# imjaegyun/Traffic-Context-Augmented-Vehicle-Trajectory-Prediction-Framework-Using-Multimodal-LLM

Hardware: AMD Instinct MI355X
Metric: trajectories/sec (higher is better)
Workload: dtype f16

## Files before the change

### traffic-context-augmented-vehicle-trajectory-prediction-framework-using-multimodal-llm_amd/csrc/attention.hip

```cpp
#include "common.hpp"
#include "philox.hpp"

namespace tcavt {

__device__ __forceinline__ f16x8 cvt8_f16(const float* v) {
  f16x8 o;
#pragma unroll
  for (int i = 0; i < 8; ++i) o[i] = static_cast<_Float16>(v[i]);
  return o;
}

__device__ __forceinline__ void halves(float x, float& lo, float& hi) {
  const auto r = __builtin_amdgcn_permlane32_swap(__float_as_uint(x), __float_as_uint(x), false, false);
  lo = __uint_as_float(r[0]);
  hi = __uint_as_float(r[1]);
}

__device__ __forceinline__ unsigned int bf16pair_to_f16pair(unsigned int k0_bits, unsigned int k1_bits) {
  const float a = fminf(fmaxf(__uint_as_float(k0_bits << 16), -65504.f), 65504.f);
  const float b = fminf(fmaxf(__uint_as_float(k1_bits << 16), -65504.f), 65504.f);
  const unsigned short ha = __builtin_bit_cast(unsigned short, static_cast<_Float16>(a));
  const unsigned short hb = __builtin_bit_cast(unsigned short, static_cast<_Float16>(b));
  return static_cast<unsigned int>(ha) | (static_cast<unsigned int>(hb) << 16);
}

template <int MAXT, bool F16>
__global__ __launch_bounds__(MAXT) void attn_causal_gqa_kernel(const bf16_t* __restrict__ qkv,
                                                              bf16_t* __restrict__ out,
                                                              const int* __restrict__ kv_len_p,
                                                              int L, int Lp, int nq, int nkv,
                                                              float scale_log2e, int ot_bytes,
                                                              float* __restrict__ lse = nullptr) {
  extern __shared__ __attribute__((aligned(16))) char smem[];
  const int group = nq / nkv;
  const int b = blockIdx.x / nkv, kvh = blockIdx.x % nkv;
  const int lane = threadIdx.x & 63;
  const int wave = __builtin_amdgcn_readfirstlane(threadIdx.x >> 6);
  const int ld = (nq + 2 * nkv) * 64;
  const int koff = nq * 64 + kvh * 64, voff = (nq + nkv) * 64 + kvh * 64;
  const int vstride = Lp + 4;
  char* Ks = smem;
  bf16_t* Vt = reinterpret_cast<bf16_t*>(smem + Lp * 128);
  const int ot_off = (Lp * 128 + 64 * (Lp + 4) * 2 + 15) & ~15;
  const bf16_t* base = qkv + (long)b * L * ld;

  const int head = kvh * group + (wave % group);
  const int qb0 = wave / group;
  const int r = lane & 31, hh = lane >> 5;
  const int nqb = (L + 31) >> 5;
  const int npair = (nqb + 1) >> 1;
  auto block_of = [&](int bi) {
    const int pr = qb0 + 2 * (bi >> 1);
    if (pr >= npair) return -1;
    const int qb = (bi & 1) ? nqb - 1 - pr : pr;
    return ((bi & 1) && qb == pr) ? -1 : qb;
  };
  auto load_q = [&](int qb, bf16x8 (&qf)[4]) {
    const int qrow = min(qb * 32 + r, L - 1);
#pragma unroll
    for (int s = 0; s < 4; ++s)
      qf[s] = *reinterpret_cast<const bf16x8*>(base + (long)qrow * ld + head * 64 + s * 16 + hh * 8);
  };
  constexpr int NPRE = 4;
  bf16x8 qpre[NPRE][4];
#pragma unroll
  for (int bi = 0; bi < NPRE; ++bi) {
    const int qb = block_of(bi);
    load_q(qb < 0 ? 0 : qb, qpre[bi]);
  }

  const int nthreads = blockDim.x;
  constexpr int KIT = 4, VIT = 2;
  auto stage_k = [&](int idx, const u32x4& v) {
    const int row = idx >> 3, c = idx & 7;
    *reinterpret_cast<u32x4*>(Ks + row * 128 + ((c ^ ((row >> 1) & 7)) << 4)) = v;
  };
  auto stage_v = [&](int idx, const u32x4& a, const u32x4& bb) {
    const int kp = idx >> 3, c = idx & 7;
    const int r0 = 2 * kp;
#pragma unroll
    for (int e = 0; e < 4; ++e) {
      unsigned int lo, hi;
      if constexpr (F16) {
        lo = (a[e] & 0xffffu) | (bb[e] << 16);
        hi = (a[e] >> 16) | (bb[e] & 0xffff0000u);
      } else {
        lo = bf16pair_to_f16pair(a[e] & 0xffffu, bb[e] & 0xffffu);
        hi = bf16pair_to_f16pair(a[e] >> 16, bb[e] >> 16);
      }
      *reinterpret_cast<unsigned int*>(Vt + (c * 8 + 2 * e) * vstride + r0) = lo;
      *reinterpret_cast<unsigned int*>(Vt + (c * 8 + 2 * e + 1) * vstride + r0) = hi;
    }
  };
  const u32x4 zero4 = {0u, 0u, 0u, 0u};
  auto load_k = [&](int idx) {
    const int row = min(idx >> 3, L - 1), c = idx & 7;
    return *reinterpret_cast<const u32x4*>(base + (long)row * ld + koff + c * 8);
  };
  auto load_v = [&](int idx, int which) {
    const int rr = min(2 * (idx >> 3) + which, L - 1), c = idx & 7;
    return *reinterpret_cast<const u32x4*>(base + (long)rr * ld + voff + c * 8);
  };
  auto krow_ok = [&](int idx) { return (idx >> 3) < L; };
  auto vrow_ok = [&](int idx, int which) { return 2 * (idx >> 3) + which < L; };
  {
    u32x4 kreg[KIT], va[VIT], vb[VIT];
#pragma unroll
    for (int it = 0; it < KIT; ++it) kreg[it] = load_k(threadIdx.x + it * nthreads);
#pragma unroll
    for (int it = 0; it < VIT; ++it) {
      va[it] = load_v(threadIdx.x + it * nthreads, 0);
      vb[it] = load_v(threadIdx.x + it * nthreads, 1);
    }
#pragma unroll
    for (int it = 0; it < KIT; ++it) {
      const int idx = threadIdx.x + it * nthreads;
      if (idx < Lp * 8) stage_k(idx, krow_ok(idx) ? kreg[it] : zero4);
    }
#pragma unroll
    for (int it = 0; it < VIT; ++it) {
      const int idx = threadIdx.x + it * nthreads;
      if (idx < (Lp >> 1) * 8) stage_v(idx, vrow_ok(idx, 0) ? va[it] : zero4, vrow_ok(idx, 1) ? vb[it] : zero4);
    }
  }
  for (int idx = threadIdx.x + KIT * nthreads; idx < Lp * 8; idx += nthreads)
    stage_k(idx, krow_ok(idx) ? load_k(idx) : zero4);
  for (int idx = threadIdx.x + VIT * nthreads; idx < (Lp >> 1) * 8; idx += nthreads)
    stage_v(idx, vrow_ok(idx, 0) ? load_v(idx, 0) : zero4, vrow_ok(idx, 1) ? load_v(idx, 1) : zero4);
  __syncthreads();

  const int kv_len = min(kv_len_p[b], L);
  const int kv_tiles = (kv_len + 31) >> 5;
  const int kswz = (r >> 1) & 7;

  auto do_block = [&](int qb, const bf16x8 (&qf)[4]) {
    const int qi = qb * 32 + r;
    f32x16 o0, o1;
#pragma unroll
    for (int i = 0; i < 16; ++i) { o0[i] = 0.f; o1[i] = 0.f; }
    float mrun = -1e30f, lrun = 0.f;

    const int ntile = min(qb + 1, kv_tiles);
    for (int kt = 0; kt < ntile; ++kt) {
      f32x16 sacc;
#pragma unroll
      for (int i = 0; i < 16; ++i) sacc[i] = 0.f;
      const char* krow = Ks + (kt * 32 + r) * 128;
#pragma unroll
      for (int s = 0; s < 4; ++s) {
        const bf16x8 kf = *reinterpret_cast<const bf16x8*>(krow + (((2 * s + hh) ^ kswz) << 4));
        if constexpr (F16)
          sacc = __builtin_amdgcn_mfma_f32_32x32x16_f16(__builtin_bit_cast(f16x8, kf), __builtin_bit_cast(f16x8, qf[s]), sacc, 0, 0, 0);
        else
          sacc = __builtin_amdgcn_mfma_f32_32x32x16_bf16(kf, qf[s], sacc, 0, 0, 0);
      }
      float p[16];
      float tmax = -1e30f;
      const bool full = (kt < qb) && (kt * 32 + 32 <= kv_len);
      if (full) {
        float rmax = fmaxf(fmaxf(sacc[0], sacc[1]), sacc[2]);
#pragma unroll
        for (int i = 3; i + 1 < 16; i += 2) rmax = fmaxf(fmaxf(rmax, sacc[i]), sacc[i + 1]);
        rmax = fmaxf(rmax, sacc[15]);
        { float a, b; halves(rmax, a, b); rmax = fmaxf(a, b); }
        const float mnew = fmaxf(mrun, rmax * scale_log2e);
        const float alpha = __builtin_amdgcn_exp2f(mrun - mnew);
        float psum = 0.f;
#pragma unroll
        for (int i = 0; i < 16; ++i) {
          p[i] = __builtin_amdgcn_exp2f(fmaf(sacc[i], scale_log2e, -mnew));
          psum += p[i];
        }
        { float a, b; halves(psum, a, b); psum = a + b; }
        lrun = lrun * alpha + psum;
        mrun = mnew;
#pragma unroll
        for (int i = 0; i < 16; ++i) { o0[i] *= alpha; o1[i] *= alpha; }
      } else {
#pragma unroll
        for (int i = 0; i < 16; ++i) {
          const int kk = kt * 32 + (i & 3) + 8 * (i >> 2) + 4 * hh;
          const bool ok = (kk <= qi) && (kk < kv_len);
          p[i] = ok ? sacc[i] * scale_log2e : -1e30f;
          tmax = fmaxf(tmax, p[i]);
        }
        { float a, b; halves(tmax, a, b); tmax = fmaxf(a, b); }
        const float mnew = fmaxf(mrun, tmax);
        const float alpha = __builtin_amdgcn_exp2f(mrun - mnew);
        float psum = 0.f;
#pragma unroll
        for (int i = 0; i < 16; ++i) {
          p[i] = (p[i] > -1e29f) ? __builtin_amdgcn_exp2f(p[i] - mnew) : 0.f;
          psum += p[i];
        }
        { float a, b; halves(psum, a, b); psum = a + b; }
        lrun = lrun * alpha + psum;
        mrun = mnew;
#pragma unroll
        for (int i = 0; i < 16; ++i) { o0[i] *= alpha; o1[i] *= alpha; }
      }
#pragma unroll
      for (int s2 = 0; s2 < 2; ++s2) {
        const f16x8 pf = cvt8_f16(&p[8 * s2]);
        const int kbase = kt * 32 + 16 * s2 + 4 * hh;
#pragma unroll
        for (int dt = 0; dt < 2; ++dt) {
          const bf16_t* vrow = Vt + (dt * 32 + r) * vstride + kbase;
          const u32x2 lo = *reinterpret_cast<const u32x2*>(vrow);
          const u32x2 hi = *reinterpret_cast<const u32x2*>(vrow + 8);
          const u32x4 vv = {lo[0], lo[1], hi[0], hi[1]};
          const f16x8 vf = __builtin_bit_cast(f16x8, vv);
          if (dt == 0) o0 = __builtin_amdgcn_mfma_f32_32x32x16_f16(vf, pf, o0, 0, 0, 0);
          else o1 = __builtin_amdgcn_mfma_f32_32x32x16_f16(vf, pf, o1, 0, 0, 0);
        }
      }
    }
    const float inv = lrun > 0.f ? 1.f / lrun : 0.f;
    if (lse && hh == 0 && qi < L) lse[((long)b * nq + head) * L + qi] = lrun > 0.f ? (mrun + __log2f(lrun)) * 0.6931471805599453f : 0.f;
    if (ot_bytes) {
      char* ot = smem + ot_off + wave * (32 * 144);
#pragma unroll
      for (int half = 0; half < 2; ++half) {
        const f32x16& o = half ? o1 : o0;
#pragma unroll
        for (int g = 0; g < 4; ++g)
          *reinterpret_cast<u32x2*>(ot + r * 144 + (half * 32 + 8 * g + 4 * hh) * 2) =
              u32x2{pack16x2<F16>(o[4 * g] * inv, o[4 * g + 1] * inv), pack16x2<F16>(o[4 * g + 2] * inv, o[4 * g + 3] * inv)};
      }
#pragma unroll
      for (int k = 0; k < 4; ++k) {
        const int row = (lane >> 3) + 8 * k, q = qb * 32 + row;
        const u32x4 v = *reinterpret_cast<const u32x4*>(ot + row * 144 + (lane & 7) * 16);
        if (q < L) *reinterpret_cast<u32x4*>(out + ((long)b * L + q) * (nq * 64) + head * 64 + (lane & 7) * 8) = v;
      }
      return;
    }
    bf16_t* orow = out + ((long)b * L + min(qi, L - 1)) * (nq * 64) + head * 64;
#pragma unroll
    for (int half = 0; half < 2; ++half) {
      const f32x16& o = half ? o1 : o0;
#pragma unroll
      for (int g = 0; g < 4; g += 2) {
        unsigned int a0 = pack16x2<F16>(o[4 * g] * inv, o[4 * g + 1] * inv), a1 = pack16x2<F16>(o[4 * g + 2] * inv, o[4 * g + 3] * inv);
        unsigned int b0 = pack16x2<F16>(o[4 * g + 4] * inv, o[4 * g + 5] * inv), b1 = pack16x2<F16>(o[4 * g + 6] * inv, o[4 * g + 7] * inv);
        auto s0 = __builtin_amdgcn_permlane32_swap(a0, b0, false, false);
        auto s1 = __builtin_amdgcn_permlane32_swap(a1, b1, false, false);
        if (qi < L) *reinterpret_cast<u32x4*>(orow + half * 32 + 8 * g + 8 * hh) = u32x4{s0[0], s1[0], s0[1], s1[1]};
      }
    }
  };

#pragma unroll
  for (int bi = 0; bi < NPRE; ++bi) {
    const int qb = block_of(bi);
    if (qb >= 0) do_block(qb, qpre[bi]);
  }
  for (int bi = NPRE;; ++bi) {
    if (qb0 + 2 * (bi >> 1) >= npair) break;
    const int qb = block_of(bi);
    if (qb < 0) continue;
    bf16x8 qf[4];
    load_q(qb, qf);
    do_block(qb, qf);
  }
}

struct b16 { bf16_t v; };
struct h16 { bf16_t v; };
template <typename T>
__device__ __forceinline__ float ldf(const T* p);
template <>
__device__ __forceinline__ float ldf<float>(const float* p) { return *p; }
template <>
__device__ __forceinline__ float ldf<b16>(const b16* p) { return bf16_to_f32(p->v); }
template <>
__device__ __forceinline__ float ldf<h16>(const h16* p) { return f16_to_f32(p->v); }
template <typename T>
__device__ __forceinline__ void stf(T* p, float x);
template <>
__device__ __forceinline__ void stf<float>(float* p, float x) { *p = x; }
template <>
__device__ __forceinline__ void stf<b16>(b16* p, float x) { p->v = f32_to_bf16(x); }
template <>
__device__ __forceinline__ void stf<h16>(h16* p, float x) { p->v = f32_to_f16(x); }

template <typename TI, typename TO>
__global__ __launch_bounds__(256) void mha_small_kernel(const TI* __restrict__ q, long ldq,
                                                        const TI* __restrict__ k, long ldk,
                                                        const TI* __restrict__ v, long ldv,
                                                        TO* __restrict__ out, long ldo,
                                                        const int* __restrict__ key_len, int Lq,
                                                        int Lk, int nh, int dh, float scale, DropoutP drop) {
  extern __shared__ __attribute__((aligned(16))) char smem[];
  float* sc = reinterpret_cast<float*>(smem);
  const int b = blockIdx.x / nh, h = blockIdx.x % nh;
  const int klen = key_len ? min(key_len[b], Lk) : Lk;
  const TI* qb = q + (long)b * Lq * ldq + h * dh;
  const TI* kb = k + (long)b * Lk * ldk + h * dh;
  const TI* vb = v + (long)b * Lk * ldv + h * dh;
  const int tid = threadIdx.x;

  const int lane = tid & 63, wave = tid >> 6;
  for (int ij = wave; ij < Lq * Lk; ij += 4) {
    const int i = ij / Lk, j = ij - i * Lk;
    float acc = 0.f;
    if (j < klen) {
      const TI* qr = qb + (long)i * ldq;
      const TI* kr = kb + (long)j * ldk;
      for (int d = lane; d < dh; d += 64) acc += ldf<TI>(qr + d) * ldf<TI>(kr + d);
      acc = wave_sum(acc);
    }
    if (lane == 0) sc[ij] = (j < klen) ? acc * scale : -1e30f;
  }
  __syncthreads();
  for (int i = wave; i < Lq; i += 4) {
    float* row = sc + i * Lk;
    float m = -1e30f;
    for (int j = lane; j < Lk; j += 64) m = fmaxf(m, row[j]);
    m = wave_max(m);
    float s = 0.f;
    for (int j = lane; j < Lk; j += 64) {
      const float e = (row[j] > -1e29f) ? __expf(row[j] - m) : 0.f;
      row[j] = e;
      s += e;
    }
    s = wave_sum(s);
    const float inv = s > 0.f ? 1.f / s : 0.f;
    for (int j = lane; j < Lk; j += 64) {
      float pj = row[j] * inv;
      if (drop.p > 0.f)
        pj *= dropout_one(drop, ((unsigned long long)blockIdx.x * Lq + i) * (unsigned long long)Lk + j);
      row[j] = pj;
    }
  }
  __syncthreads();
  for (int id = tid; id < Lq * dh; id += 256) {
    const int i = id / dh, d = id - i * dh;
    const float* row = sc + i * Lk;
    float acc = 0.f;
    for (int j = 0; j < klen; ++j) acc += row[j] * ldf<TI>(vb + (long)j * ldv + d);
    TO* o = out + ((long)b * Lq + i) * ldo + h * dh + d;
    stf<TO>(o, acc);
  }
}

template <typename TI, typename TO>
__global__ __launch_bounds__(256) void mha_lds_kernel(const TI* __restrict__ q, long ldq,
                                                      const TI* __restrict__ k, long ldk,
                                                      const TI* __restrict__ v, long ldv,
                                                      TO* __restrict__ out, long ldo,
                                                      const int* __restrict__ key_len, int Lq, int Lk,
                                                      int nh, int dh, float scale, DropoutP drop) {
  extern __shared__ __attribute__((aligned(16))) char smem[];
  const int ds = dh + 1;
  float* Qs = reinterpret_cast<float*>(smem);
  float* Ks = Qs + Lq * ds;
  float* Vs = Ks + Lk * ds;
  float* sc = Vs + Lk * ds;
  const int b = blockIdx.x / nh, h = blockIdx.x % nh;
  const int klen = key_len ? min(key_len[b], Lk) : Lk;
  const TI* qb = q + (long)b * Lq * ldq + h * dh;
  const TI* kb = k + (long)b * Lk * ldk + h * dh;
  const TI* vb = v + (long)b * Lk * ldv + h * dh;
  const int tid = threadIdx.x, lane = tid & 63, wave = tid >> 6;
  for (int id = tid; id < Lq * dh; id += 256) {
    const int i = id / dh, d = id - i * dh;
    Qs[i * ds + d] = ldf<TI>(qb + (long)i * ldq + d);
  }
  for (int id = tid; id < Lk * dh; id += 256) {
    const int j = id / dh, d = id - j * dh;
    Ks[j * ds + d] = ldf<TI>(kb + (long)j * ldk + d);
    Vs[j * ds + d] = ldf<TI>(vb + (long)j * ldv + d);
  }
  __syncthreads();
  for (int ij = tid; ij < Lq * Lk; ij += 256) {
    const int i = ij / Lk, j = ij - i * Lk;
    float acc = 0.f;
    if (j < klen) {
      const float* qr = Qs + i * ds;
      const float* kr = Ks + j * ds;
      for (int d = 0; d < dh; ++d) acc = fmaf(qr[d], kr[d], acc);
    }
    sc[ij] = (j < klen) ? acc * scale : -1e30f;
  }
  __syncthreads();
  for (int i = wave; i < Lq; i += 4) {
    float* row = sc + i * Lk;
    float m = -1e30f;
    for (int j = lane; j < Lk; j += 64) m = fmaxf(m, row[j]);
    m = wave_max(m);
    float s = 0.f;
    for (int j = lane; j < Lk; j += 64) {
      const float e = (row[j] > -1e29f) ? __expf(row[j] - m) : 0.f;
      row[j] = e;
      s += e;
    }
    s = wave_sum(s);
    const float inv = s > 0.f ? 1.f / s : 0.f;
    for (int j = lane; j < Lk; j += 64) {
      float pj = row[j] * inv;
      if (drop.p > 0.f)
        pj *= dropout_one(drop, ((unsigned long long)blockIdx.x * Lq + i) * (unsigned long long)Lk + j);
      row[j] = pj;
    }
  }
  __syncthreads();
  for (int id = tid; id < Lq * dh; id += 256) {
    const int i = id / dh, d = id - i * dh;
    const float* row = sc + i * Lk;
    float acc = 0.f;
    for (int j = 0; j < klen; ++j) acc = fmaf(row[j], Vs[j * ds + d], acc);
    TO* o = out + ((long)b * Lq + i) * ldo + h * dh + d;
    stf<TO>(o, acc);
  }
}

}

using namespace tcavt;

extern "C" int tcavt_attn_causal_gqa(const void* qkv, void* out, const int32_t* kv_len, int B, int L,
                                     int nq, int nkv, float scale, int dtype16, tcavt_stream_t stream) {
  return tcavt_attn_causal_gqa_lse(qkv, out, nullptr, kv_len, B, L, nq, nkv, scale, dtype16, stream);
}

extern "C" int tcavt_attn_causal_gqa_lse(const void* qkv, void* out, float* lse, const int32_t* kv_len, int B, int L,
                                         int nq, int nkv, float scale, int dtype16, tcavt_stream_t stream) {
  TCAVT_CHECK_ARG(qkv && out && kv_len, "attn_causal_gqa: null pointer");
  TCAVT_CHECK_ARG(is16(dtype16), "attn_causal_gqa: dtype16 must be TCAVT_BF16 or TCAVT_F16");
  TCAVT_CHECK_ARG(B > 0 && L > 0 && L <= 544, "attn_causal_gqa: L=%d must be in [1, 544]", L);
  TCAVT_CHECK_ARG(nkv > 0 && nq % nkv == 0 && nq / nkv <= 8, "attn_causal_gqa: nq/nkv must be an integer <= 8");
  TCAVT_CHECK_ARG(aligned16(qkv) && aligned16(out), "attn_causal_gqa: unaligned pointer");
  const int Lp = (L + 31) & ~31;
  int lds = Lp * 128 + 64 * (Lp + 4) * 2;
  const int group = nq / nkv;
  const bool small = 2 * group * 64 <= 512;
  int ot_bytes = 2 * group * 32 * 144;
  if (((lds + 15) & ~15) + ot_bytes <= 160 * 1024 - 256) lds = ((lds + 15) & ~15) + ot_bytes;
  else ot_bytes = 0;
  const bool f16 = dtype16 == TCAVT_F16;
  const void* fns[4] = {reinterpret_cast<const void*>(attn_causal_gqa_kernel<1024, false>),
                        reinterpret_cast<const void*>(attn_causal_gqa_kernel<512, false>),
                        reinterpret_cast<const void*>(attn_causal_gqa_kernel<1024, true>),
                        reinterpret_cast<const void*>(attn_causal_gqa_kernel<512, true>)};
  const int which = (f16 ? 2 : 0) + (small ? 1 : 0);
  static bool attr_set[4] = {false, false, false, false};
  if (!attr_set[which]) {
    hipError_t e = hipFuncSetAttribute(fns[which], hipFuncAttributeMaxDynamicSharedMemorySize, 160 * 1024 - 256);
    if (e != hipSuccess) {
      set_error("attn_causal_gqa: hipFuncSetAttribute failed: %s", hipGetErrorString(e));
      return TCAVT_ERR_HIP;
    }
    attr_set[which] = true;
  }
#define TCAVT_ATTN(MAXT, F)                                                                                       \
  hipLaunchKernelGGL((attn_causal_gqa_kernel<MAXT, F>), dim3(B * nkv), dim3(2 * group * 64), lds,                  \
                     static_cast<hipStream_t>(stream), static_cast<const bf16_t*>(qkv), static_cast<bf16_t*>(out), \
                     kv_len, L, Lp, nq, nkv, scale * 1.4426950408889634f, ot_bytes, lse)
  if (which == 0) TCAVT_ATTN(1024, false);
  else if (which == 1) TCAVT_ATTN(512, false);
  else if (which == 2) TCAVT_ATTN(1024, true);
  else TCAVT_ATTN(512, true);
#undef TCAVT_ATTN
  TCAVT_CHECK_LAUNCH("attn_causal_gqa");
  return TCAVT_OK;
}

extern "C" int tcavt_mha(const void* q, int64_t ldq, const void* k, int64_t ldk, const void* v,
                         int64_t ldv, void* out, int64_t ldo, const int32_t* key_len, int B, int Lq,
                         int Lk, int nh, int dh, float scale, int in_dtype, int out_dtype, float dropout_p,
                         uint64_t dropout_seed, uint32_t dropout_site, tcavt_stream_t stream) {
  TCAVT_CHECK_ARG(dropout_p >= 0.f && dropout_p < 1.f, "mha: dropout_p must be in [0, 1)");
  const DropoutP drop = make_dropout(dropout_p, dropout_seed, dropout_site);
  TCAVT_CHECK_ARG(q && k && v && out, "mha: null pointer");
  TCAVT_CHECK_ARG(B > 0 && Lq > 0 && Lk > 0 && nh > 0 && dh > 0, "mha: bad shape");
  const long lds = (long)Lq * Lk * 4;
  TCAVT_CHECK_ARG(lds <= 64 * 1024, "mha: Lq*Lk*4 = %ld bytes exceeds the 64 KiB score buffer", lds);
  hipStream_t s = static_cast<hipStream_t>(stream);
  dim3 grid(B * nh), block(256);
  const long lds_all = ((long)(Lq + 2 * Lk) * (dh + 1) + (long)Lq * Lk) * 4;
  const bool whole = lds_all <= 60 * 1024;
  const long lds_use = whole ? lds_all : lds;
#define TCAVT_MHA(TI, TO)                                                                                          \
  do {                                                                                                             \
    if (whole)                                                                                                     \
      hipLaunchKernelGGL((mha_lds_kernel<TI, TO>), grid, block, lds_use, s, (const TI*)q, ldq, (const TI*)k, ldk, \
                         (const TI*)v, ldv, (TO*)out, ldo, key_len, Lq, Lk, nh, dh, scale, drop);                  \
    else                                                                                                           \
      hipLaunchKernelGGL((mha_small_kernel<TI, TO>), grid, block, lds_use, s, (const TI*)q, ldq, (const TI*)k, ldk, \
                         (const TI*)v, ldv, (TO*)out, ldo, key_len, Lq, Lk, nh, dh, scale, drop);                  \
  } while (0)
#define TCAVT_MHA_IN(TI)                                  \
  do {                                                    \
    if (out_dtype == TCAVT_F32) TCAVT_MHA(TI, float);     \
    else if (out_dtype == TCAVT_BF16) TCAVT_MHA(TI, b16); \
    else TCAVT_MHA(TI, h16);                              \
  } while (0)
  TCAVT_CHECK_ARG((in_dtype == TCAVT_F32 || is16(in_dtype)) && (out_dtype == TCAVT_F32 || is16(out_dtype)),
                  "mha: bad dtype %d/%d", in_dtype, out_dtype);
  if (in_dtype == TCAVT_F32) TCAVT_MHA_IN(float);
  else if (in_dtype == TCAVT_BF16) TCAVT_MHA_IN(b16);
  else TCAVT_MHA_IN(h16);
#undef TCAVT_MHA_IN
#undef TCAVT_MHA
  TCAVT_CHECK_LAUNCH("mha");
  return TCAVT_OK;
}
```

### traffic-context-augmented-vehicle-trajectory-prediction-framework-using-multimodal-llm_amd/csrc/gemm_w4.hpp

```cpp
#pragma once
#include "gemm_epilogue.hpp"

namespace tcavt {

template <bool F16>
__device__ __forceinline__ void mfma_agpr(f32x4& c, const bf16x8& a, const bf16x8& b) {
  if constexpr (F16) asm volatile("v_mfma_f32_16x16x32_f16 %0, %1, %2, %0" : "+a"(c) : "v"(a), "v"(b));
  else asm volatile("v_mfma_f32_16x16x32_bf16 %0, %1, %2, %0" : "+a"(c) : "v"(a), "v"(b));
}

constexpr bool w4_pers_ok(int epi, bool deep) {
  return epi != EPI_ROPE && !(deep && epi == EPI_GENERIC);
}

template <int EPI, bool F16, int BN = 256, bool DEEP = false, int B2R = (BN == 256 ? 2 : 4)>
__global__ __launch_bounds__(256) void gemm_bf16_w4_kernel(GemmP p) {
  constexpr int BM = 256, NW = 4;
  constexpr int WN_ = BN == 256 ? 2 : 1, WM_ = NW / WN_;
  constexpr int TM = BM / WM_ / 16, TN = BN / WN_ / 16;
  static_assert(TM + TN == 16, "the fragment pipeline assumes 16 fragment loads per 32-deep K-step");
  constexpr int TILE_BYTES = (BM + BN) * 128;
  constexpr int NP = (BM + BN) / 32;
  constexpr int NB2 = B2R * TM;
  static_assert(!DEEP || (TM == 8 && TN == 8), "DEEP is laid out for the 2x2-wave form");
  constexpr int EARLY = NB2 / 4;
  constexpr int SPREAD = (TM * TN) / (NP - EARLY);
  extern __shared__ __attribute__((aligned(16))) char smem[];

  const int lane = threadIdx.x & 63;
  const int wave = __builtin_amdgcn_readfirstlane(threadIdx.x >> 6);
  const int wm = wave / WN_, wn = wave % WN_;
  constexpr bool RS = EPI == EPI_SILU || EPI == EPI_SILU_SAVE || EPI == EPI_ROPE;
  float* const rs_base = reinterpret_cast<float*>(smem + 2 * TILE_BYTES);
  int rs_sel = 0;
  constexpr bool PERS_OK = w4_pers_ok(EPI, DEEP);
  const bool pers = PERS_OK && p.pers_tiles > 0;
  const int total_tiles = pers ? p.pers_tiles : (int)gridDim.x;
  int vb = blockIdx.x;
  int tile_m, tile_n;
  block_to_tile(p, tile_m, tile_n, vb, total_tiles);
  int m0 = tile_m * BM, n0 = tile_n * BN;

  const int rl = lane >> 3;
  const int csw = (lane & 7) ^ (((wave & 1) * 4 + (rl >> 1)) & 7);
  const bf16_t* srcA = p.A + (long)(m0 + wave * 8 + rl) * p.lda + csw * 8;
  const bf16_t* srcW = p.W + (long)(n0 + wave * 8 + rl) * p.ldw + csw * 8;
  bool has_next = pers && vb + (int)gridDim.x < total_tiles;
  int nm0 = m0, nn0 = n0;
  const bf16_t* nxtA = srcA;
  const bf16_t* nxtW = srcW;
  auto locate_next = [&]() {
    if (has_next) {
      int tm, tn;
      block_to_tile(p, tm, tn, vb + (int)gridDim.x, total_tiles);
      nm0 = tm * BM;
      nn0 = tn * BN;
      nxtA = p.A + (long)(nm0 + wave * 8 + rl) * p.lda + csw * 8;
      nxtW = p.W + (long)(nn0 + wave * 8 + rl) * p.ldw + csw * 8;
    }
  };
  locate_next();
  const long stepA = 32 * p.lda, stepW = 32 * p.ldw;
  constexpr bool HASK2 = EPI == EPI_ROPE;
  const bf16_t* srcA2 = nullptr;
  const bf16_t* srcW2 = nullptr;
  long stepA2 = 0, stepW2 = 0;
  const int nt1 = p.K >> 6;
  int nt = nt1;
  auto locate_k2 = [&]() {
    if constexpr (HASK2) {
      if (p.K2 > 0) {
        srcA2 = p.A2 + (long)(m0 + wave * 8 + rl) * p.lda2 + csw * 8;
        srcW2 = p.W2 + (long)(n0 + wave * 8 + rl) * p.ldw2 + csw * 8;
      }
    }
  };
  if constexpr (HASK2) {
    if (p.K2 > 0) {
      stepA2 = 32 * p.lda2;
      stepW2 = 32 * p.ldw2;
      nt += p.K2 >> 6;
    }
  }
  locate_k2();

  struct Src {
    const bf16_t* a;
    const bf16_t* w;
    long sa, sw;
  };
  auto tsrc = [&](int t) -> Src {
    if constexpr (PERS_OK) {
      if (t >= nt && has_next) return Src{nxtA + (t - nt) * 64, nxtW + (t - nt) * 64, stepA, stepW};
    }
    t = min(t, nt - 1);
    if constexpr (HASK2) {
      if (t >= nt1) return Src{srcA2 + (t - nt1) * 64, srcW2 + (t - nt1) * 64, stepA2, stepW2};
    }
    return Src{srcA + t * 64, srcW + t * 64, stepA, stepW};
  };
  auto piece = [&](int buf, const Src& s, int r) {
    char* dst = smem + buf * TILE_BYTES + (r * NW + wave) * 1024;
    if (r < 8)
      glds16(s.a + r * s.sa, dst);
    else
      glds16(s.w + (r - 8) * s.sw, dst);
  };

  const int fsw = (lane >> 1) & 7;
  const int off0 = ((lane >> 4) ^ fsw) * 16;
  const int off1 = ((4 + (lane >> 4)) ^ fsw) * 16;
  const int xrow = (wm * TM * 16 + (lane & 15)) * 128;
  const int wrow = (BM + wn * TN * 16 + (lane & 15)) * 128;

  f32x4 acc[TN][TM];
#pragma unroll
  for (int i = 0; i < TN; ++i)
#pragma unroll
    for (int j = 0; j < TM; ++j) acc[i][j] = f32x4{0.f, 0.f, 0.f, 0.f};

  bf16x8 w0[TN], x0[TM], w1[TN], x1[TM];
  auto ldx = [&](const char* base, int off, int j) { return *reinterpret_cast<const bf16x8*>(base + xrow + j * 2048 + off); };
  auto ldw = [&](const char* base, int off, int i) { return *reinterpret_cast<const bf16x8*>(base + wrow + i * 2048 + off); };

  if constexpr (RS) {
    if (p.rs_part) rs_base[threadIdx.x] = row_rscale(p, m0 + threadIdx.x);
  }
  {
    const Src s0 = tsrc(0);
#pragma unroll
    for (int r = 0; r < NP; ++r) piece(0, s0, r);
  }
  __syncthreads();
  Src sn1 = tsrc(1);
  if constexpr (DEEP) {
#pragma unroll
    for (int r = 0; r < NP; ++r) piece(1, sn1, r);
  } else if (nt > 1) {
#pragma unroll
    for (int r = 0; r < EARLY; ++r) piece(1, sn1, r);
  }
#pragma unroll
  for (int j = 0; j < TM; ++j) x0[j] = ldx(smem, off0, j);
#pragma unroll
  for (int i = 0; i < TN; ++i) w0[i] = ldw(smem, off0, i);

  int cur = 0;
  auto ktile = [&](int t) {
    const char* base = smem + cur * TILE_BYTES;
    const char* nbase = smem + (cur ^ 1) * TILE_BYTES;
    Src sn2;
    int koff2 = 0;
    bool second2 = false, into_next2 = false;
#pragma unroll
    for (int i = 0; i < TN; ++i) {
#pragma unroll
      for (int j = 0; j < TM; ++j) {
        mfma_agpr<F16>(acc[i][j], w0[i], x0[j]);
        const int idx = i * TM + j;
        if (idx < 32 && (idx & 1) == 0) {
          const int f = idx >> 1;
          if (f < TM) x1[f] = ldx(base, off1, f);
          else w1[f - TM] = ldw(base, off1, f - TM);
        }
        if constexpr (DEEP) {
          if (idx == 0) {
            into_next2 = PERS_OK && has_next && t + 2 >= nt;
            const int tt = into_next2 ? t + 2 - nt : min(t + 2, nt - 1);
            second2 = HASK2 && !into_next2 && tt >= nt1;
            koff2 = (second2 ? tt - nt1 : tt) * 64;
          }
          if (idx == 3) sn2.a = (into_next2 ? nxtA : second2 ? srcA2 : srcA) + koff2;
          if (idx == 6) sn2.w = (into_next2 ? nxtW : second2 ? srcW2 : srcW) + koff2;
          if (idx == 9) {
            sn2.sa = second2 ? stepA2 : stepA;
            sn2.sw = second2 ? stepW2 : stepW;
          }
          if (idx == 39) asm volatile("s_waitcnt lgkmcnt(0)\n\ts_barrier" ::: "memory");
          if (idx >= 43 && (idx & 3) == 3) piece(cur, sn2, (idx - 43) / 4);
        } else {
          if (idx % SPREAD == SPREAD - 1 && EARLY + idx / SPREAD < NP) piece(cur ^ 1, sn1, EARLY + idx / SPREAD);
        }
      }
    }
#pragma unroll
    for (int i = 0; i < TN - B2R; ++i)
#pragma unroll
      for (int j = 0; j < TM; ++j) {
        mfma_agpr<F16>(acc[i][j], w1[i], x1[j]);
        const int idx = i * TM + j;
        if constexpr (DEEP) {
          if ((idx & 3) == 3 && 6 + idx / 4 < NP) piece(cur, sn2, 6 + idx / 4);
          continue;
        }
        if (idx == 0) {
          into_next2 = PERS_OK && has_next && t + 2 >= nt;
          const int tt = into_next2 ? t + 2 - nt : min(t + 2, nt - 1);
          second2 = HASK2 && !into_next2 && tt >= nt1;
          koff2 = (second2 ? tt - nt1 : tt) * 64;
        }
        if (idx == 3) sn2.a = (into_next2 ? nxtA : second2 ? srcA2 : srcA) + koff2;
        if (idx == 6) sn2.w = (into_next2 ? nxtW : second2 ? srcW2 : srcW) + koff2;
        if (idx == 9) {
          sn2.sa = second2 ? stepA2 : stepA;
          sn2.sw = second2 ? stepW2 : stepW;
        }
      }
    if (DEEP) asm volatile("s_waitcnt vmcnt(%0) lgkmcnt(0)\n\ts_barrier" ::"n"(NP) : "memory");
    else __syncthreads();
#pragma unroll
    for (int i = TN - B2R; i < TN; ++i) {
#pragma unroll
      for (int j = 0; j < TM; ++j) {
        mfma_agpr<F16>(acc[i][j], w1[i], x1[j]);
        const int idx = (i - (TN - B2R)) * TM + j;
        if (TM == TN && idx < TM) {
          x0[idx] = ldx(nbase, off0, idx);
          w0[idx] = ldw(nbase, off0, idx);
        }
        if (TM != TN && idx < 16) {
          if (idx < TM) x0[idx] = ldx(nbase, off0, idx);
          else w0[idx - TM] = ldw(nbase, off0, idx - TM);
        }
        if (!DEEP && (idx & 3) == 3 && (idx >> 2) < EARLY) piece(cur, sn2, idx >> 2);
      }
    }
    if (t == nt - 1) asm volatile("s_nop 15\n\ts_nop 15" ::: "memory");
    cur ^= 1;
    sn1 = sn2;
  };
  for (;;) {
    for (int t = 0; t < nt; ++t) ktile(t);
    asm volatile("s_nop 15\n\ts_nop 15" ::: "memory");
#pragma unroll
    for (int i = 0; i < TN; ++i)
#pragma unroll
      for (int j = 0; j < TM; ++j) asm volatile("" : "+a"(acc[i][j]));
    const int em0 = m0, en0 = n0;
    const bool cont = PERS_OK && has_next;
    if (cont) {
      vb += gridDim.x;
      if constexpr (RS) {
        if (p.rs_part) rs_base[(rs_sel ^ 1) * 256 + threadIdx.x] = row_rscale(p, nm0 + threadIdx.x);
      }
      m0 = nm0;
      n0 = nn0;
      srcA = nxtA;
      srcW = nxtW;
      locate_k2();
      has_next = vb + (int)gridDim.x < total_tiles;
      locate_next();
    }
    __builtin_amdgcn_sched_barrier(0);
    gemm_epilogue<TM, TN, EPI, true, F16>(p, acc, em0 + wm * TM * 16, en0 + wn * TN * 16, lane,
                                          (RS && p.rs_part) ? rs_base + rs_sel * 256 + wm * TM * 16 : nullptr);
    if (!cont) {
      if constexpr (DEEP) asm volatile("s_waitcnt vmcnt(0)" ::: "memory");
      break;
    }
    rs_sel ^= 1;
#pragma unroll
    for (int i = 0; i < TN; ++i)
#pragma unroll
      for (int j = 0; j < TM; ++j) {
        acc[i][j] = f32x4{0.f, 0.f, 0.f, 0.f};
        asm volatile("" : "+a"(acc[i][j]));
      }
    asm volatile("s_nop 7" ::: "memory");
  }
}

template <bool F16>
static bool silu16_ok(const GemmP& p) {
  return p.out_kind == (F16 ? TCAVT_F16 : TCAVT_BF16) && (p.ldc & 7) == 0;
}

template <int EPI, bool F16, int BN = 256, bool DEEP = false>
static int launch_w4(const GemmP& p0, hipStream_t stream) {
  if constexpr (EPI == EPI_SILU || EPI == EPI_SILU_SAVE) {
    if (!silu16_ok<F16>(p0)) {
      set_error("gemm_bf16(w4): the SiLU epilogue of the 4-wave kernel writes the 16-bit operand type with ldc %% 8 == 0");
      return TCAVT_ERR_ARG;
    }
  }
  if constexpr (EPI == EPI_SILUBWD) {
    if (p0.out_kind != (F16 ? TCAVT_F16 : TCAVT_BF16) || (p0.ldc & 7) || (p0.ldaux & 7) || p0.aux == nullptr || p0.ldc < 2 * p0.N ||
        p0.ldaux < 2 * p0.N) {
      set_error("gemm_bf16(w4): SILU_BWD needs silu_preact, 16-bit output of the operand type, ldc / ld_preact %% 8 == 0 and >= 2 N");
      return TCAVT_ERR_ARG;
    }
  }
  if constexpr (EPI == EPI_ROPE) {
    if (p0.ldc & 7) {
      set_error("gemm_bf16(w4): the RoPE epilogue of the 4-wave kernel needs ldc %% 8 == 0");
      return TCAVT_ERR_ARG;
    }
  }
  if constexpr (EPI == EPI_NORM16) {
    if (p0.ldc & 7) {
      set_error("gemm_bf16(w4): the in-place 16-bit residual epilogue of the 4-wave kernel needs ldc %% 8 == 0");
      return TCAVT_ERR_ARG;
    }
  }
  GemmP p = p0;
  p.tiles_m = p.M / 256;
  p.tiles_n = p.N / BN;
  p.xcd_gx = choose_xcd_partition(p);
  constexpr int lds = 2 * (256 + BN) * 128 + 2048;
  auto kfn = gemm_bf16_w4_kernel<EPI, F16, BN, DEEP>;
  static bool attr_set = false;
  if (!attr_set) {
    hipError_t e = hipFuncSetAttribute(reinterpret_cast<const void*>(kfn),
                                       hipFuncAttributeMaxDynamicSharedMemorySize, lds);
    if (e != hipSuccess) {
      set_error("gemm_bf16(w4): hipFuncSetAttribute(%d B LDS) failed: %s", lds, hipGetErrorString(e));
      return TCAVT_ERR_HIP;
    }
    attr_set = true;
  }
  const int tiles = p.tiles_m * p.tiles_n;
  static const bool no_pers = getenv("TCAVT_GEMM_NO_PERSIST") != nullptr;
  static const int n_cu = [] {
    int dev = 0, n = 0;
    if (hipGetDevice(&dev) != hipSuccess || hipDeviceGetAttribute(&n, hipDeviceAttributeMultiprocessorCount, dev) != hipSuccess) n = 256;
    return n / 8 * 8;
  }();
  int wgs = tiles;
  p.pers_tiles = 0;
  if (w4_pers_ok(EPI, DEEP) && !no_pers && n_cu >= 8 && tiles > n_cu && p.K + p.K2 >= 128) {
    p.pers_tiles = tiles;
    wgs = n_cu;
  }
  dim3 grid(wgs), block(256);
  hipLaunchKernelGGL(kfn, grid, block, lds, stream, p);
  TCAVT_CHECK_LAUNCH("gemm_bf16(w4)");
  return TCAVT_OK;
}

}
```

Baseline: 2085.

## Enable persistent scheduling for RoPE GEMM and reorder attention Q prefetch

Allows the persistent-tile GEMM path to be used for the RoPE epilogue, which was previously excluded, and restructures the K2 source-pointer selection through a candidate struct, likely to keep register pressure manageable. The RoPE k-tile loop is kept rolled. Persistence is now also skipped when a second K segment exists but the first K is short. In attention, the Q fragment prefetch is moved after the K/V global loads so that the K/V loads are issued first. The changes risk higher register pressure and different scheduling in the RoPE kernel.

```diff
diff --git a/traffic-context-augmented-vehicle-trajectory-prediction-framework-using-multimodal-llm_amd/csrc/attention.hip b/traffic-context-augmented-vehicle-trajectory-prediction-framework-using-multimodal-llm_amd/csrc/attention.hip
--- a/traffic-context-augmented-vehicle-trajectory-prediction-framework-using-multimodal-llm_amd/csrc/attention.hip
+++ b/traffic-context-augmented-vehicle-trajectory-prediction-framework-using-multimodal-llm_amd/csrc/attention.hip
@@ -63,12 +63,6 @@
   };
   constexpr int NPRE = 4;
   bf16x8 qpre[NPRE][4];
-#pragma unroll
-  for (int bi = 0; bi < NPRE; ++bi) {
-    const int qb = block_of(bi);
-    load_q(qb < 0 ? 0 : qb, qpre[bi]);
-  }
-
   const int nthreads = blockDim.x;
   constexpr int KIT = 4, VIT = 2;
   auto stage_k = [&](int idx, const u32x4& v) {
@@ -111,6 +105,11 @@
     for (int it = 0; it < VIT; ++it) {
       va[it] = load_v(threadIdx.x + it * nthreads, 0);
       vb[it] = load_v(threadIdx.x + it * nthreads, 1);
+    }
+#pragma unroll
+    for (int bi = 0; bi < NPRE; ++bi) {
+      const int qb = block_of(bi);
+      load_q(qb < 0 ? 0 : qb, qpre[bi]);
     }
 #pragma unroll
     for (int it = 0; it < KIT; ++it) {
diff --git a/traffic-context-augmented-vehicle-trajectory-prediction-framework-using-multimodal-llm_amd/csrc/gemm_w4.hpp b/traffic-context-augmented-vehicle-trajectory-prediction-framework-using-multimodal-llm_amd/csrc/gemm_w4.hpp
--- a/traffic-context-augmented-vehicle-trajectory-prediction-framework-using-multimodal-llm_amd/csrc/gemm_w4.hpp
+++ b/traffic-context-augmented-vehicle-trajectory-prediction-framework-using-multimodal-llm_amd/csrc/gemm_w4.hpp
@@ -10,7 +10,7 @@
 }
 
 constexpr bool w4_pers_ok(int epi, bool deep) {
-  return epi != EPI_ROPE && !(deep && epi == EPI_GENERIC);
+  return !(deep && epi == EPI_GENERIC);
 }
 
 template <int EPI, bool F16, int BN = 256, bool DEEP = false, int B2R = (BN == 256 ? 2 : 4)>
@@ -89,14 +89,22 @@
     const bf16_t* w;
     long sa, sw;
   };
+  struct Cand {
+    const bf16_t *a_main, *a_k2, *a_next, *w_main, *w_k2, *w_next;
+    long sa_main, sa_k2, sw_main, sw_k2;
+  };
   auto tsrc = [&](int t) -> Src {
+    if constexpr (HASK2) {
+      const Cand cd{srcA, srcA2, nxtA, srcW, srcW2, nxtW, stepA, stepA2, stepW, stepW2};
+      if (PERS_OK && t >= nt && has_next) return Src{cd.a_next + (t - nt) * 64, cd.w_next + (t - nt) * 64, cd.sa_main, cd.sw_main};
+      t = min(t, nt - 1);
+      if (t >= nt1) return Src{cd.a_k2 + (t - nt1) * 64, cd.w_k2 + (t - nt1) * 64, cd.sa_k2, cd.sw_k2};
+      return Src{cd.a_main + t * 64, cd.w_main + t * 64, cd.sa_main, cd.sw_main};
+    }
     if constexpr (PERS_OK) {
       if (t >= nt && has_next) return Src{nxtA + (t - nt) * 64, nxtW + (t - nt) * 64, stepA, stepW};
     }
     t = min(t, nt - 1);
-    if constexpr (HASK2) {
-      if (t >= nt1) return Src{srcA2 + (t - nt1) * 64, srcW2 + (t - nt1) * 64, stepA2, stepW2};
-    }
     return Src{srcA + t * 64, srcW + t * 64, stepA, stepW};
   };
   auto piece = [&](int buf, const Src& s, int r) {
@@ -150,6 +158,8 @@
     const char* base = smem + cur * TILE_BYTES;
     const char* nbase = smem + (cur ^ 1) * TILE_BYTES;
     Src sn2;
+    [[maybe_unused]] Cand cd{};
+    if constexpr (HASK2) cd = Cand{srcA, srcA2, nxtA, srcW, srcW2, nxtW, stepA, stepA2, stepW, stepW2};
     int koff2 = 0;
     bool second2 = false, into_next2 = false;
 #pragma unroll
@@ -170,11 +180,19 @@
             second2 = HASK2 && !into_next2 && tt >= nt1;
             koff2 = (second2 ? tt - nt1 : tt) * 64;
           }
-          if (idx == 3) sn2.a = (into_next2 ? nxtA : second2 ? srcA2 : srcA) + koff2;
-          if (idx == 6) sn2.w = (into_next2 ? nxtW : second2 ? srcW2 : srcW) + koff2;
+          if (idx == 3) {
+            if constexpr (HASK2) sn2.a = (into_next2 ? cd.a_next : second2 ? cd.a_k2 : cd.a_main) + koff2;
+            else sn2.a = (into_next2 ? nxtA : second2 ? srcA2 : srcA) + koff2;
+          }
+          if (idx == 6) {
+            if constexpr (HASK2) sn2.w = (into_next2 ? cd.w_next : second2 ? cd.w_k2 : cd.w_main) + koff2;
+            else sn2.w = (into_next2 ? nxtW : second2 ? srcW2 : srcW) + koff2;
+          }
           if (idx == 9) {
-            sn2.sa = second2 ? stepA2 : stepA;
-            sn2.sw = second2 ? stepW2 : stepW;
+            if constexpr (HASK2) sn2.sa = second2 ? cd.sa_k2 : cd.sa_main;
+            else sn2.sa = second2 ? stepA2 : stepA;
+            if constexpr (HASK2) sn2.sw = second2 ? cd.sw_k2 : cd.sw_main;
+            else sn2.sw = second2 ? stepW2 : stepW;
           }
           if (idx == 39) asm volatile("s_waitcnt lgkmcnt(0)\n\ts_barrier" ::: "memory");
           if (idx >= 43 && (idx & 3) == 3) piece(cur, sn2, (idx - 43) / 4);
@@ -199,11 +217,19 @@
           second2 = HASK2 && !into_next2 && tt >= nt1;
           koff2 = (second2 ? tt - nt1 : tt) * 64;
         }
-        if (idx == 3) sn2.a = (into_next2 ? nxtA : second2 ? srcA2 : srcA) + koff2;
-        if (idx == 6) sn2.w = (into_next2 ? nxtW : second2 ? srcW2 : srcW) + koff2;
+        if (idx == 3) {
+          if constexpr (HASK2) sn2.a = (into_next2 ? cd.a_next : second2 ? cd.a_k2 : cd.a_main) + koff2;
+          else sn2.a = (into_next2 ? nxtA : second2 ? srcA2 : srcA) + koff2;
+        }
+        if (idx == 6) {
+          if constexpr (HASK2) sn2.w = (into_next2 ? cd.w_next : second2 ? cd.w_k2 : cd.w_main) + koff2;
+          else sn2.w = (into_next2 ? nxtW : second2 ? srcW2 : srcW) + koff2;
+        }
         if (idx == 9) {
-          sn2.sa = second2 ? stepA2 : stepA;
-          sn2.sw = second2 ? stepW2 : stepW;
+          if constexpr (HASK2) sn2.sa = second2 ? cd.sa_k2 : cd.sa_main;
+          else sn2.sa = second2 ? stepA2 : stepA;
+          if constexpr (HASK2) sn2.sw = second2 ? cd.sw_k2 : cd.sw_main;
+          else sn2.sw = second2 ? stepW2 : stepW;
         }
       }
     if (DEEP) asm volatile("s_waitcnt vmcnt(%0) lgkmcnt(0)\n\ts_barrier" ::"n"(NP) : "memory");
@@ -230,7 +256,12 @@
     sn1 = sn2;
   };
   for (;;) {
-    for (int t = 0; t < nt; ++t) ktile(t);
+    if constexpr (EPI == EPI_ROPE) {
+#pragma unroll 1
+      for (int t = 0; t < nt; ++t) ktile(t);
+    } else {
+      for (int t = 0; t < nt; ++t) ktile(t);
+    }
     asm volatile("s_nop 15\n\ts_nop 15" ::: "memory");
 #pragma unroll
     for (int i = 0; i < TN; ++i)
@@ -327,7 +358,7 @@
   }();
   int wgs = tiles;
   p.pers_tiles = 0;
-  if (w4_pers_ok(EPI, DEEP) && !no_pers && n_cu >= 8 && tiles > n_cu && p.K + p.K2 >= 128) {
+  if (w4_pers_ok(EPI, DEEP) && !no_pers && n_cu >= 8 && tiles > n_cu && p.K + p.K2 >= 128 && (p.K2 == 0 || p.K >= 128)) {
     p.pers_tiles = tiles;
     wgs = n_cu;
   }
```

Result: no change. 2084 (-0.0%).
